# PolusAI/nyxus

Hardware: AMD Instinct MI355X
Metric: ROIs/sec (*ALL_GLCM*+*ALL_INTENSITY*, 1024^2 tiles) (higher is better)
Workload: dtype f64; 1 GPU; *ALL_GLCM*+*ALL_INTENSITY*, coarse_gray_depth=8, 4 angles, d=1, 1000 synthetic 1024x1024 tiles/GPU x 196 ROIs/tile (disk r=30, 2821 px, bbox 61x61), intensities U[1,4095]; reduce stage on pre-assembled ROI clouds resident in HBM; n_columns=185

## Files before the change

### nyxus_amd/csrc/nyxhip_dispatch.hip

```cpp
#include "nyxhip_ctx.h"

using namespace nyxhip;

namespace {

uint32_t align16(uint32_t v) { return (v + 15u) & ~15u; }

void gabor_filter(double* Gex, double f0, double sig2lam, double gamma, double theta, double fi, int n)
{
    const double lambda = 2 * M_PI / f0, cos_theta = cos(theta), sin_theta = sin(theta), sig = sig2lam * lambda;
    std::vector<double> tx(n + 1), ty(n + 1);
    tx[0] = (n % 2 > 0) ? -((n - 1) / 2) : -(n / 2);
    for (int x = 1; x < n; x++) tx[x] = tx[x - 1] + 1;
    ty[0] = tx[0];
    for (int y = 1; y < n; y++) ty[y] = ty[y - 1] + 1;
    double sum = 0;
    for (int y = 0; y < n; y++)
        for (int x = 0; x < n; x++) {
            double xte = tx[x] * cos_theta + ty[y] * sin_theta;
            double yte = ty[y] * cos_theta - tx[x] * sin_theta;
            double rte = xte * xte + gamma * gamma * yte * yte;
            double ge = exp(-1 * rte / (2 * sig * sig));
            double argm = xte * f0 + fi;
            int idx = y * n * 2 + x * 2;
// ... 1069 lines not shown
        const bool after_all = (mask & kBehindIntensity) && (mask & NYXHIP_FAM_GLCM);
        if (after_all) lane_join.join();
        if (int mrc = launch_contour_families(ctx, b, mask, s, d_out, ld, max_px, max_area, max_side, !after_all))
            return mrc;
    }
    return NYXHIP_OK;
}

}

namespace nyxhip {

int use_lane(nyxhip_ctx* ctx, int lane, hipStream_t* st)
{
    if (!ctx->lane_stream[lane]) {
        static const bool no_prio = [] { const char* e = getenv("NYXHIP_NO_LANE_PRIORITY"); return e && *e && *e != '0'; }();
        int lo = 0, hi = 0;
        if (no_prio || hipDeviceGetStreamPriorityRange(&lo, &hi) != hipSuccess) lo = hi = 0;
        HIP_TRY(ctx, hipStreamCreateWithPriority(&ctx->lane_stream[lane], hipStreamNonBlocking, hi));
        HIP_TRY(ctx, hipEventCreateWithFlags(&ctx->lane_done[lane], hipEventDisableTiming));
    }
    if (!ctx->lane_used[lane]) {
        HIP_TRY(ctx, hipStreamWaitEvent(ctx->lane_stream[lane], ctx->lane_fork, 0));
        ctx->lane_used[lane] = true;
    }
    *st = ctx->lane_stream[lane];
    return NYXHIP_OK;
}

size_t large_budget(size_t dflt)
{
    const char* const be = getenv("NYXHIP_LARGE_BUDGET_MB");
    return be && atoll(be) > 0 ? (size_t)atoll(be) << 20 : dflt;
}

uint32_t pow2ceil(uint32_t v)
{
    uint32_t p = 1;
    while (p < v) p <<= 1;
    return p;
}

int make_layout(uint32_t mask, const nyxhip_settings* s, int n_cols, uint32_t max_px, uint32_t max_area,
                uint32_t max_range, LdsLayout& L, std::string& why, size_t cap, uint32_t vmax, bool wide_only)
{
    memset(&L, 0, sizeof(L));
    const bool do_int = mask & NYXHIP_FAM_INTENSITY, do_glcm = mask & NYXHIP_FAM_GLCM;
    const bool spill = cap != 0;
    if (!spill) cap = roi_features_max_lds();
    uint32_t off = 0;
    L.out = off;
    L.red = off; off = align16(off + 8u * kWaves * 8);
    L.stat = off; off = align16(off + 8u * 16);
    L.lb100 = off; off = align16(off + 4u * 104);
    uint32_t n_hist = (uint32_t)abs(s->grey_depth);
    L.lbc = off; off = align16(off + 4u * (do_int ? n_hist + 8 : 8));
    const uint32_t fixed = off;
    const uint32_t kCountCapMax = spill ? (1u << 22) : 16384u, kCountCapMixed = 4096;
    const bool radix = do_int && wide_only && !spill;
    if (radix) {
        L.count_cap = 0;
        L.sort_cap = max_px ? max_px : 1;
    } else if (do_int) {
        if ((uint64_t)max_range + 1 <= kCountCapMax) {
            L.count_cap = (max_range + 1 + 63u) & ~63u;
            L.sort_cap = max_px ? max_px : 1;
        } else {
            L.count_cap = kCountCapMixed;
            L.sort_cap = pow2ceil(max_px ? max_px : 1);
        }
    }
    L.dense_cap = do_glcm ? max_area : 0;
    L.dense = off;
    {
        const int gi = s->ibsi ? 0 : s->grey_depth;
        const bool c16_pred = do_int && max_px < 65536u && (uint64_t)max_range + 1 <= kCountCapMax && max_range < 65536u;
        const bool split_pred = do_glcm && !spill && gi > 0 && gi <= 16 && s->glcm_n_angles > 0;
        L.dense8 = ((c16_pred || !do_int) && split_pred) ? 1u : 0u;
    }
    {
        const int gi = s->ibsi ? 0 : s->grey_depth;
        const bool c16_pred = (!do_int || (uint64_t)max_range + 1 <= kCountCapMax) && max_range < 65536u;
        L.g16 = (do_glcm && !spill && gi > 16 && gi <= 64 && max_px < 32768u && c16_pred && s->glcm_n_angles > 0) ? 1u : 0u;
        if (L.g16) L.dense8 = 1;
    }
    if ((L.dense8 ? 1ull : 2ull) * L.dense_cap > cap) { why = "ROI bounding box of " + std::to_string(max_area) + " px exceeds the LDS-resident plane"; return NYXHIP_ERR_ROI_TOO_LARGE; }
    uint32_t plane_bytes = L.dense8 ? 1u * L.dense_cap + 64 + 8 : 2u * L.dense_cap + 8;
    const uint32_t g16_scratch = L.g16 ? 8u * ((uint32_t)s->grey_depth + kMaxAngles * 128u) : 0u;
    if (plane_bytes < g16_scratch) plane_bytes = g16_scratch;
    off = align16(off + plane_bytes);
    if (do_glcm) {
        const int greyInfo = s->ibsi ? 0 : s->grey_depth;
        L.lvl_cap = greyInfo < 0 ? (uint32_t)(-greyInfo) : 0;
        L.lvlmap = off; off = align16(off + 2u * (L.lvl_cap + 8));
    }
    const uint32_t shared0 = off;
    L.val = off;
    L.cnt16 = (do_int && max_px < 65536u && (uint64_t)max_range + 1 <= kCountCapMax && max_range < 65536u) ? 1u : 0u;
    L.radix_k16 = (radix && max_range < 65536u) ? 1u : 0u;
    if ((L.cnt16 ? 2ull : 4ull) * L.sort_cap > cap) { why = "ROI pixel count " + std::to_string(max_px) + " exceeds the LDS-resident value buffer"; return NYXHIP_ERR_ROI_TOO_LARGE; }
    if (L.radix_k16) off = align16(off + 2u * 2u * ((L.sort_cap + 7u) & ~7u) + 16);
    else off = align16(off + (L.cnt16 ? 2u : 4u) * L.sort_cap + 16);
    L.cnt = off; off = align16(off + (L.cnt16 ? 2u : 4u) * L.count_cap + 16);
    if (radix) {
        if (8ull * L.sort_cap > cap) { why = "ROI pixel count " + std::to_string(max_px) + " exceeds the LDS-resident sort buffers"; return NYXHIP_ERR_ROI_TOO_LARGE; }
        L.radix = off; off = align16(off + (L.radix_k16 ? 0u : 4u * L.sort_cap) + 4u * (kWaves * 256 + kWaves) + 16);
    }
    if (do_glcm && L.g16) {
        const uint32_t ng = (uint32_t)s->grey_depth, cellsw = ((ng + 1) * ((ng + 3) & ~1u)) / 2;
        L.ng_cap = ng; L.app = 4;
        uint32_t goff = shared0;
        L.P = goff; goff = align16(goff + 4u * 4u * cellsw);
        L.gscr = L.dense;
        if (goff > off) off = goff;
    } else if (do_glcm) {
        const int greyInfo = s->ibsi ? 0 : s->grey_depth;
        auto glcm_bytes = [&](uint32_t ng, uint32_t app) -> size_t {
            return (size_t)align16(4u * app * ng * ng) + 8ull * (25ull * ng + 128);
        };
        uint32_t ng;
        if (greyInfo != 0) {
            ng = (uint32_t)abs(greyInfo);
            if (fixed + 2ull * (L.lvl_cap + 8) + glcm_bytes(ng, 1) > cap) {
                why = "GLCM grey depth " + std::to_string(ng) + " too large for the LDS-resident co-occurrence matrix";
                return NYXHIP_ERR_UNSUPPORTED;
            }
        } else {
            if (vmax != 0) {
                ng = vmax < 8 ? 8 : vmax;
                if (shared0 + glcm_bytes(ng, 1) > cap) {
                    why = "IBSI GLCM matrix order " + std::to_string(ng) + " too large for the LDS-resident co-occurrence matrix";
                    return NYXHIP_ERR_UNSUPPORTED;
                }
            } else {
                ng = 128;
                while (ng > 8 && shared0 + glcm_bytes(ng, 1) > cap) ng >>= 1;
            }
        }
        uint32_t app = 4;
        while (app > 1 && ((!spill && 4ull * app * ng * ng > 64 * 1024) || shared0 + glcm_bytes(ng, app) > cap)) app >>= 1;
        L.ng_cap = ng;
        L.app = app;
        uint32_t goff = shared0;
        L.P = goff; goff = align16(goff + 4u * app * (ng <= 16 ? (ng + 1) * (ng + 1) : ng * ng));
        L.gscr = goff; goff = align16(goff + 8u * (25u * ng + 128));
        if (goff > off) off = goff;
    }
    if (L.dense8) {
        const uint32_t dsz = align16(plane_bytes);
        L.out += dsz; L.red += dsz; L.stat += dsz; L.lb100 += dsz; L.lbc += dsz;
        L.dense = 0;
        if (L.g16) L.gscr = 0;
    }
    if (spill) {
        const uint32_t esz = L.cnt16 ? 2u : 4u;
        const uint64_t sz_val = align16(esz * L.sort_cap + 16), sz_cnt = do_int ? (uint64_t)esz * L.count_cap + 32 : 0;
        const uint64_t sz_dense = 2ull * L.dense_cap + 24, sz_lvl = do_glcm ? 2ull * (L.lvl_cap + 8) + 16 : 0;
        const uint64_t ngc = L.ng_cap, sz_P = do_glcm ? 4ull * L.app * (ngc <= 16 ? (ngc + 1) * (ngc + 1) : ngc * ngc) + 16 : 0;
        const uint64_t sz_g = do_glcm ? 8ull * (25ull * ngc + 128) + 16 : 0;
        const uint64_t kLdsMax = 60 * 1024;
        uint64_t o = fixed;
        const bool p_lds = do_glcm && o + sz_P + sz_g <= kLdsMax;
        if (p_lds) { L.P = (uint32_t)o; o = (o + sz_P + 15) & ~15ull; L.gscr = (uint32_t)o; o = (o + sz_g + 15) & ~15ull; }
        const bool c_lds = do_int && o + sz_cnt <= kLdsMax;
        if (c_lds) { L.cnt = (uint32_t)o; o = (o + sz_cnt + 15) & ~15ull; }
        const bool l_lds = do_glcm && o + sz_lvl <= kLdsMax;
        if (l_lds) { L.lvlmap = (uint32_t)o; o = (o + sz_lvl + 15) & ~15ull; }
        L.gs_lds_bytes = (uint32_t)o;
        if (do_glcm && !l_lds) { L.lvlmap = (uint32_t)o; o = (o + sz_lvl + 15) & ~15ull; }
        L.dense = (uint32_t)o; o = (o + sz_dense + 15) & ~15ull;
        L.val = (uint32_t)o; o = (o + sz_val + 15) & ~15ull;
        if (do_int && !c_lds) { L.cnt = (uint32_t)o; o = (o + sz_cnt + 15) & ~15ull; }
        if (do_glcm && !p_lds) { L.P = (uint32_t)o; o = (o + sz_P + 15) & ~15ull; L.gscr = (uint32_t)o; o = (o + sz_g + 15) & ~15ull; }
        if (o > cap) { why = "ROI too large for the global workspace (2 GiB of offsets per workgroup)"; return NYXHIP_ERR_ROI_TOO_LARGE; }
        off = (uint32_t)o;
    }
    L.total = off;
    if (L.total > cap) {
        why = "ROI too large for the LDS-resident path (" + std::to_string(L.total) + " B of LDS needed; max_px=" +
              std::to_string(max_px) + ", max_bbox_area=" + std::to_string(max_area) + ")";
        return NYXHIP_ERR_ROI_TOO_LARGE;
    }
    return NYXHIP_OK;
}

int ensure_stage(nyxhip_ctx* ctx, size_t bytes)
{
    HIP_TRY(ctx, ctx->d_stage.reserve(bytes, nullptr, bytes + bytes / 4 + (1 << 20)));
    return NYXHIP_OK;
}

int check_status(nyxhip_ctx* ctx)
{
    int two[2] = {0, 0};
    HIP_TRY(ctx, hipMemcpy(two, ctx->d_status.p, 2 * sizeof(int), hipMemcpyDeviceToHost));
    const int st = two[0];
    if (ctx->census_pending) {
        ctx->census_small = (uint32_t)two[1]; ctx->census_total = ctx->census_pending; ctx->census_pending = 0;
    }
    if (two[1]) HIP_TRY(ctx, hipMemsetAsync(ctx->d_status.as<int>() + 1, 0, sizeof(int), ctx->stream()));
    if (st != 0) {
        int zero = 0;
        HIP_TRY(ctx, hipMemcpy(ctx->d_status.p, &zero, sizeof(int), hipMemcpyHostToDevice));
// ... 88 lines not shown
```

### nyxus_amd/csrc/roi_features.hip

```cpp
#include <hip/hip_runtime.h>
#include <type_traits>
#include <algorithm>
#include <cstdlib>
#include <cstdio>
#include "device_math.h"
#include "roi_kernel.h"
#include "launch_util.h"
#include "glcm_rows.h"
#include "glcm_w64.h"
#include "intensity_close.h"
#include "sort_lds.h"
#include "../../include/nyxhip.h"

namespace nyxhip {


enum { S_MEAN = 0, S_P10, S_P90, S_MEDIAN, S_MODE, S_NG };


template <int NW> __device__ __forceinline__ double xw_chain(const double* s_red, int k)
{
    return NW == 1 ? s_red[k] : ((s_red[k] + s_red[8 + k]) + s_red[16 + k]) + s_red[24 + k];
}
template <int NW> __device__ __forceinline__ double xw_pairs(const double* s_red, int k)
// ... 642 lines not shown
    glcm_w64_tail<NG>(Ng, lane, rc, cc, dc, pxpy_c, csum, sum_p, inv_sum_p, pcol, prow, pxmy, pxpy, ent, hxy1c, hxy2, asm_i, cmax, f);
}

#ifdef NYX_STAMP
#define STAMP(i)                                                                          \
    do {                                                                                  \
        unsigned long long t__ = __builtin_readcyclecounter();                            \
        if (tid == 0 && A.stamps) atomicAdd(&A.stamps[i], t__ - t_prev__);                \
        t_prev__ = __builtin_readcyclecounter();                                          \
    } while (0)
#elif defined(NYX_EXIT_AT)
#define STAMP(i) do { if ((i) == NYX_EXIT_AT) return; } while (0)
#else
#define STAMP(i) do { } while (0)
#endif

__constant__ const double kPctFrac[8] = {0.01, 0.1, 0.25, 0.75, 0.9, 0.99, 0.5, 0.5};

typedef __attribute__((address_space(3))) uint8_t lds_u8_t;

typedef const __attribute__((address_space(4))) RoiArgs KArgs;
__device__ __forceinline__ KArgs* late_kernarg()
{
    KArgs* p = (KArgs*)__builtin_amdgcn_kernarg_segment_ptr();
    asm volatile("" : "+s"(p));
    return p;
}
template <bool LATE>
struct KView {
    const RoiArgs& a;
    KArgs* p;
    __device__ __forceinline__ explicit KView(const RoiArgs& a_) : a(a_), p(LATE ? late_kernarg() : nullptr) {}
    __device__ __forceinline__ auto operator->() const
    {
        if constexpr (LATE) return p;
        else return &a;
    }
};
template <bool GS, bool C16, bool SPLIT, bool D8, int FAM = 0, int TIER = 4, bool G16 = false, int WIN = 2, int NW = 4, bool DEFER_P = false>
__device__ __forceinline__ void roi_features_body(const RoiArgs& A, const uint64_t slot)
{
    static_assert((NW == 4 && NW == kMaxAngles) || (NW == 8 && G16 && FAM == 4), "one workgroup of four waves per ROI (and a wave per GLCM angle)");
    constexpr int BS = NW * 64;
    extern __shared__ __attribute__((aligned(16))) unsigned char lds_raw[];
    unsigned char* const lds = GS ? A.sp.scratch + (size_t)blockIdx.x * A.sp.stride : lds_raw;
    const int tid = (int)threadIdx.x, lane = tid & 63, wave = __builtin_amdgcn_readfirstlane(tid >> 6);
    uint64_t roi;
    if (!roi_of_slot(A.sp, slot, A.n_roi, roi))
        return;

    auto reg = [&](uint32_t o) -> unsigned char* { return (GS && o < A.L.gs_lds_bytes) ? lds_raw + o : lds + o; };
    double* s_red = (double*)reg(A.L.red);
    double* s_stat = (double*)reg(A.L.stat);
    uint32_t* s_lb100 = (uint32_t*)reg(A.L.lb100);
    uint32_t* s_lbc = (uint32_t*)reg(A.L.lbc);
    uint32_t* s_val = (uint32_t*)(lds + A.L.val);
    using dense_t = typename std::conditional<D8, uint8_t, uint16_t>::type;
    dense_t* s_dense = (dense_t*)(lds + (D8 ? 0u : A.L.dense));
    uint16_t* s_lvlmap = (uint16_t*)reg(A.L.lvlmap);
    uint32_t* s_P = (uint32_t*)reg(A.L.P);
    double* s_g = (double*)reg(A.L.gscr);

    const uint64_t off = A.px_offset[roi];
    const uint32_t n = (uint32_t)(A.px_offset[roi + 1] - off);
    const uint32_t w = A.bbox_w[roi], h = A.bbox_h[roi];
    const uint32_t area = w * h;
    const uint32_t vmin = A.min_inten[roi], vmax = A.max_inten[roi];
    if (!roi_in_launch(A.sp, n, w, h, vmax - vmin))
        return;
    if (vmax - vmin < A.sp.min_range || (A.sp.max_range != 0u && vmax - vmin > A.sp.max_range))
        return;
    constexpr bool FAST = FAM == 1 || FAM == 3;
    constexpr int kRowsTag = 16 + TIER * 4 + (C16 ? 2 : 0) + (D8 ? 1 : 0);
    const bool do_int = FAM == 1 || FAM == 2 || (FAM == 0 && (A.mask & NYXHIP_FAM_INTENSITY) != 0);
    const bool do_glcm = FAM == 1 || FAM == 3 || FAM == 4 || (FAM == 0 && (A.mask & NYXHIP_FAM_GLCM) != 0);
    double* const out_row = A.out + roi * A.ld;
#ifdef NYX_STAMP
    unsigned long long t_prev__ = __builtin_readcyclecounter();
#endif

    const uint32_t range = vmax - vmin;
    const bool use_count = C16 ? do_int : (do_int && A.L.count_cap != 0 && range < A.L.count_cap);
    if (C16 && do_int && range >= A.L.count_cap) {
        if (tid == 0) atomicCAS(A.status, 0, NYXHIP_ERR_ROI_TOO_LARGE);
        return;
    }
    uint32_t* s_cnt = (uint32_t*)reg(A.L.cnt);
    uint32_t P2 = 1;
    while (P2 < n)
        P2 <<= 1;
    const bool radix = !C16 && A.L.radix != 0;
    const bool k16 = radix && A.L.radix_k16 != 0;
    if (n == 0 || (do_int && ((use_count || radix) ? n : P2) > A.L.sort_cap) || (do_glcm && area > A.L.dense_cap)) {
        if (SPLIT && A.glcm_ng && tid == 0)
            A.glcm_ng[roi] = 0;
        if (n != 0 && A.sp.defer_large)
            return;
        if (tid == 0 && n != 0)
            atomicCAS(A.status, 0, NYXHIP_ERR_ROI_TOO_LARGE);
        for (int c = tid; c < A.n_cols; c += BS)
            out_row[c] = __longlong_as_double(0x7ff8000000000000LL);
        return;
    }

    const int greyInfo = A.ibsi ? 0 : A.grey_depth;
    if (FAST) __builtin_assume(greyInfo > 0 && greyInfo <= 16);
    if (G16) __builtin_assume(greyInfo > 16 && greyInfo <= 64);
// ... 277 lines not shown
        if ((unsigned long long)n * vmax < (1ull << 32))
            sum = wave_sum_t<uint32_t>((uint32_t)sum);
        else
            sum = wave_sum_u64(sum);
        if (C16) {
            const uint32_t lo24 = wave_sum_t<uint32_t>((uint32_t)sumsq & 0xFFFFFFu), hi = wave_sum_t<uint32_t>((uint32_t)(sumsq >> 24));
            sumsq = ((unsigned long long)hi << 24) + lo24;
        } else
            sumsq = wave_sum_u64(sumsq);
        if (lane == 0) {
            s_red[wave * 8 + 0] = (double)sum;
            s_red[wave * 8 + 1] = (double)sumsq;
        }
        grp_sync<GS, NW>();
        const bool blank = (vmin == 0 && vmax == 0);
#if defined(NYX_NO_FUSED) || defined(NYX_NO_DEFER)
        constexpr bool DEFER = false;
#else
        constexpr bool DEFER = DEFER_P && C16 && !GS;
#endif
        const bool defer = DEFER && !blank;
        double* const rec = DEFER ? B->close_rec + roi * kCloseRec : nullptr;
        if (tid == 0) {
            double tot = 0, totsq = 0;
            for (int wv = 0; wv < NW; wv++) {
                tot += s_red[wv * 8 + 0];
                totsq += s_red[wv * 8 + 1];
            }
            const double mean = tot / dn;
            s_stat[S_MEAN] = mean;
            if (FAST)
                s_stat[S_NG] = bin_pixel(vmin, vmin, vmax, B->glcm_grey_depth) == bin_pixel(vmax, vmin, vmax, B->glcm_grey_depth) ? 1.0 : 0.0;
            if (defer) {
                rec[CR_TOT] = tot;
                rec[CR_TOTSQ] = totsq;
            } else {
                close_sums(RowColumns{o}, dn, vmin, vmax, tot, totsq, mean, B->slide_min && B->slide_max,
                           [&] { return B->slide_max[roi] - B->slide_min[roi]; }, blank);
            }
        }
        grp_sync<GS, NW>();
        const double mean = s_stat[S_MEAN];
        STAMP(2);

        const double binW100 = (double)range / 100.;
        const uint32_t nb = (uint32_t)B->n_hist;
        auto idx100 = [=](uint32_t v) -> int {
            double realIdx = (double)(v - vmin) / binW100;
            return (realIdx != realIdx) ? 0 : (int)realIdx;
        };

        const uint32_t Q = ((range + 1 + NW * 512 - 1) / (NW * 512)) * 512;
        uint32_t* const s_woff = (uint32_t*)(s_stat + 8);
        if (use_count) {
            uint32_t carry = 0, best_c = 0, best_i = 0;
            const uint32_t base = wave * Q;
            if (C16) {
                uint32_t kk[8] = {0, 0, 0, 0, 0, 0, 0, 0};
                uint32_t inv = 0xFFFFu - (base + 8u * (uint32_t)lane);
                uint4* src = (uint4*)((uint16_t*)s_cnt + base + 8u * (uint32_t)lane);
                uint32_t i = base + 8u * (uint32_t)lane;
                for (uint32_t t = 0; t < Q; t += 512, i += 512, inv -= 512, src += 64) {
                    uint4 pk = make_uint4(0, 0, 0, 0);
                    const bool live = i <= range;
                    if (live) pk = *src;
                    kk[0] = max(kk[0], (pk.x << 16) | inv); kk[1] = max(kk[1], (pk.x & 0xFFFF0000u) | inv);
                    kk[2] = max(kk[2], (pk.y << 16) | inv); kk[3] = max(kk[3], (pk.y & 0xFFFF0000u) | inv);
                    kk[4] = max(kk[4], (pk.z << 16) | inv); kk[5] = max(kk[5], (pk.z & 0xFFFF0000u) | inv);
                    kk[6] = max(kk[6], (pk.w << 16) | inv); kk[7] = max(kk[7], (pk.w & 0xFFFF0000u) | inv);
                    const uint32_t A0 = pk.x + (pk.x << 16), A1 = pk.y + (pk.y << 16), A2 = pk.z + (pk.z << 16), A3 = pk.w + (pk.w << 16);
                    const uint32_t T = ((A0 + A1) + (A2 + A3)) >> 16;
                    const uint32_t sc = wave_scan_u32(T);
                    const uint32_t excl = carry + sc - T;
                    const uint32_t o0 = A0 + (excl | (excl << 16));
                    const uint32_t o1 = A1 + __builtin_amdgcn_perm(o0, o0, 0x03020302u);
                    const uint32_t o2 = A2 + __builtin_amdgcn_perm(o1, o1, 0x03020302u);
                    const uint32_t o3 = A3 + __builtin_amdgcn_perm(o2, o2, 0x03020302u);
                    if (live)
                        *src = make_uint4(o0, o1, o2, o3);
                    carry += readlane63(sc);
                }
#pragma unroll
                for (int q = 1; q < 8; q++) kk[q] -= (uint32_t)q;
                const uint32_t key = wave_max_u32(max(max(max(kk[0], kk[1]), max(kk[2], kk[3])), max(max(kk[4], kk[5]), max(kk[6], kk[7]))));
                best_c = key >> 16;
                best_i = 0xFFFFu - (key & 0xFFFFu);
            } else
            for (uint32_t t = 0; t < Q; t += 256) {
                uint32_t i = base + t + 4 * lane;
                uint4 c4 = make_uint4(0, 0, 0, 0);
                if (C16) {
                    if (i <= range) {
                        const uint2 pk = *(const uint2*)((const uint16_t*)s_cnt + i);
                        c4 = make_uint4(pk.x & 0xFFFFu, pk.x >> 16, pk.y & 0xFFFFu, pk.y >> 16);
                    }
                } else if (i + 3 <= range)
                    c4 = *(const uint4*)&s_cnt[i];
                else {
                    if (i <= range) c4.x = s_cnt[i];
                    if (i + 1 <= range) c4.y = s_cnt[i + 1];
                    if (i + 2 <= range) c4.z = s_cnt[i + 2];
                }
                if (c4.x > best_c) { best_c = c4.x; best_i = i; }
                if (c4.y > best_c) { best_c = c4.y; best_i = i + 1; }
                if (c4.z > best_c) { best_c = c4.z; best_i = i + 2; }
                if (c4.w > best_c) { best_c = c4.w; best_i = i + 3; }
                c4.y += c4.x; c4.z += c4.y; c4.w += c4.z;
                const uint32_t sc = wave_scan_u32(c4.w);
                uint32_t excl = carry + sc - c4.w;
                c4.x += excl; c4.y += excl; c4.z += excl; c4.w += excl;
                if (C16) {
                    if (i <= range)
                        *(uint2*)((uint16_t*)s_cnt + i) = make_uint2(c4.x | (c4.y << 16), c4.z | (c4.w << 16));
                } else if (i + 3 <= range)
                    *(uint4*)&s_cnt[i] = c4;
                else {
                    if (i <= range) s_cnt[i] = c4.x;
                    if (i + 1 <= range) s_cnt[i + 1] = c4.y;
                    if (i + 2 <= range) s_cnt[i + 2] = c4.z;
                }
                carry += readlane63(sc);
            }
            if (!C16) {
                const uint32_t mc_w = wave_max_u32(best_c);
                const uint32_t cand = best_c == mc_w ? best_i : 0xFFFFFFFFu;
                best_i = ~wave_max_u32(~cand);
                best_c = mc_w;
            }
            if (lane == 0) {
                s_red[wave * 8 + 0] = (double)carry;
                s_red[wave * 8 + 1] = (double)best_c;
                s_red[wave * 8 + 2] = (double)best_i;
            }
            grp_sync<GS, NW>();
            if (tid == 0) {
                uint32_t mc = 0, mi = 0;
                for (int wv = 0; wv < NW; wv++) {
                    uint32_t c = (uint32_t)s_red[wv * 8 + 1], i = (uint32_t)s_red[wv * 8 + 2];
                    if (c > mc) { mc = c; mi = i; }
                }
                const uint32_t woff1 = (uint32_t)s_red[0], woff2 = woff1 + (NW > 1 ? (uint32_t)s_red[8] : 0u), woff3 = woff2 + (NW > 1 ? (uint32_t)s_red[16] : 0u);
                s_woff[0] = 0; s_woff[1] = woff1; s_woff[2] = woff2; s_woff[3] = woff3;
                s_stat[S_MODE] = (double)(vmin + mi);
            }
            grp_sync<GS, NW>();
        } else if (radix) {
            if (k16) {
                uint16_t* const kb = (uint16_t*)s_val + ((B->L.sort_cap + 7u) & ~7u);
                s_val = (uint32_t*)radix_sort<GS, NW, uint16_t>((uint16_t*)s_val, kb, (uint32_t*)reg(B->L.radix), n, 0u, range, tid);
            } else {
                uint32_t* const s_rdx = (uint32_t*)reg(B->L.radix);
                s_val = radix_sort<GS, NW, uint32_t>(s_val, s_rdx, s_rdx + B->L.sort_cap, n, vmin, range, tid);
            }
        } else {
            bitonic_sort<GS, NW>(s_val, P2, tid);
        }
        STAMP(3);
        auto SV = [=](uint32_t i) -> uint32_t { return k16 ? vmin + (uint32_t)((const uint16_t*)s_val)[i] : s_val[i]; };
        auto cum = [=](uint32_t i) -> uint32_t {
            const uint32_t wq = (uint32_t)(i >= Q) + (uint32_t)(i >= 2 * Q) + (uint32_t)(i >= 3 * Q);
            return (C16 ? (uint32_t)((const uint16_t*)s_cnt)[i] : s_cnt[i]) + s_woff[wq];
        };

#ifdef NYX_NO_FUSED
        constexpr bool FUSED = false;
#else
        constexpr bool FUSED = C16 && !GS;
#endif
        double acc[6] = {0, 0, 0, 0, 0, 0};
        if (!FUSED || blank) {
            if (!blank) {
                for (uint32_t i = tid; i < n; i += BS) {
                    double d = (double)(C16 ? vmin + ((const uint16_t*)s_val)[i] : SV(i)) - mean;
                    double d2 = d * d;
                    acc[0] += fabs(d);
                    acc[1] += d2;
                    acc[2] += d2 * d;
                    acc[3] += d2 * d2;
                    acc[4] += d2 * d2 * d;
                    acc[5] += d2 * d2 * d2;
                }
                block_sum<6, GS, NW>(acc, s_red, tid);
            }
            if (tid == 0)
                close_central<CovDiv::ieee>(RowColumns{o}, acc, n, dn, mean, blank);
        }
        STAMP(4);

        if (!blank) {
            auto bin_bound = [&](auto is100_t, const uint32_t b) -> uint32_t {
                constexpr bool is100 = decltype(is100_t)::value;
                uint32_t lo;
                if (use_count) {
                    auto bin_of = [=](uint32_t dd) -> uint32_t {
                        return is100 ? (uint32_t)idx100(vmin + dd) : to_grayscale(vmin + dd, vmin, range, nb);
                    };
                    uint32_t d;
                    if (range < 65536u) {
                        const double Wl = is100 ? binW100 : (double)range / (double)nb;
                        const double P = (double)b * Wl;
                        const uint32_t m = (uint32_t)(P + 0.5);
                        d = (uint32_t)P + 1;
                        if (b == 0)
                            d = 0;
                        else if (fabs(P - (double)m) < 1e-6)
                            d = bin_of(m) >= b ? m : m + 1;
                    } else {
                        double edge = is100 ? (double)b * binW100 : (double)b * (double)range / (double)nb;
                        d = edge >= (double)range + 1.0 ? range + 1 : (uint32_t)edge;
                        while (d > 0 && bin_of(d - 1) >= b) d--;
                        while (d <= range && bin_of(d) < b) d++;
                    }
                    lo = d > 0 ? cum(d - 1) : 0u;
                } else {
                    uint32_t hi = n;
                    lo = 0;
                    while (lo < hi) {
                        uint32_t mid = (lo + hi) >> 1;
                        uint32_t v = SV(mid);
                        uint32_t idx = is100 ? (uint32_t)idx100(v) : to_grayscale(v, vmin, range, nb);
                        if (idx < b) lo = mid + 1; else hi = mid;
// ... 23 lines not shown
                for (int d = 32; d > 0; d >>= 1) {
                    uint32_t oc = __shfl_down(best_c, d, 64), ov = __shfl_down(best_v, d, 64);
                    if (oc > best_c || (oc == best_c && ov < best_v)) { best_c = oc; best_v = ov; }
                }
                if (lane == 0) {
                    s_red[wave * 8 + 0] = (double)best_c;
                    s_red[wave * 8 + 1] = (double)best_v;
                }
                grp_sync<GS, NW>();
                if (tid == 0) {
                    uint32_t mc = 0, mv = 0;
                    for (int wv = 0; wv < NW; wv++) {
                        uint32_t c = (uint32_t)s_red[wv * 8 + 0], v = (uint32_t)s_red[wv * 8 + 1];
                        if (c > mc || (c == mc && v < mv)) { mc = c; mv = v; }
                    }
                    s_stat[S_MODE] = (double)mv;
                }
            }
            STAMP(6);

            if (NW == 1 || wave == 0) {
                const int g = lane >> 3, sub = lane & 7;
                const double mycnt = dn * kPctFrac[g];
                const uint32_t k = g < 6 ? (uint32_t)mycnt : (g == 6 || n / 2 == 0) ? n / 2 : n / 2 - 1;
                uint32_t xv;
                if (use_count) {
                    uint32_t lom1 = 0xFFFFFFFFu, span = range + 1;
                    while (span > 1) {
                        const uint32_t B = (span + 7) >> 3;
                        uint32_t i = mad_u24_su((uint32_t)sub + 1, B, lom1);
                        if (i > range) i = range;
                        const unsigned long long hit = __ballot(cum(i) > k);
                        const uint32_t half = lane < 32 ? (uint32_t)hit : (uint32_t)(hit >> 32);
                        const uint32_t first = (uint32_t)__builtin_ctz(((half >> (lane & 24)) & 0xFFu) | 0x80u);
                        lom1 = mad_u24_su(first, B, lom1);
                        span = B;
                    }
                    xv = vmin + lom1 + 1;
                } else
                    xv = SV(k);
                const uint32_t win = min((uint32_t)idx100(xv), 99u);
                const uint32_t bb = win + (uint32_t)sub;
                uint32_t bnd = 0;
                if (g < 6 && sub < 2)
                    bnd = bb < 100u ? bin_bound(std::true_type{}, bb) : n;
                const uint32_t rs = bnd, bi = wave_rol1(bnd) - rs;
                const double pv = (mycnt - (double)rs) * binW100 / (double)bi + (double)vmin + binW100 * (double)win;
                static_assert(I_P10 == I_P01 + 1 && I_P25 == I_P01 + 2 && I_P75 == I_P01 + 3 && I_P90 == I_P01 + 4 && I_P99 == I_P01 + 5, "P01 .. P99 are adjacent columns");
                if (g < 6 && sub == 0)
                    o[I_P01 + g] = pv;
                const double p10 = readlane_f64(pv, 8), p90 = readlane_f64(pv, 32);
                const double p25 = DEFER ? 0.0 : readlane_f64(pv, 16), p75 = DEFER ? 0.0 : readlane_f64(pv, 24);
                const uint32_t hi_v = (uint32_t)__builtin_amdgcn_readlane((int)xv, 48), lo_v = (uint32_t)__builtin_amdgcn_readlane((int)xv, 56);
                if (lane == 0) {
                    if (!DEFER)
                        close_quartiles(RowColumns{o}, p25, p75);
                    s_stat[S_P10] = p10;
                    s_stat[S_P90] = p90;
                    if (FUSED) {
                        uint32_t lox = 0x80000000u, span = 0;
                        if (p10 <= p90 && p90 >= (double)vmin && p10 <= (double)vmax) {
                            const double cl = ceil(p10), fl = floor(p90);
                            const uint32_t lo_b = cl <= (double)vmin ? vmin : (uint32_t)cl, hi_b = fl >= (double)vmax ? vmax : (uint32_t)fl;
                            if (lo_b <= hi_b) { lox = lo_b - vmin; span = hi_b - lo_b; }
                        }
                        const bool empty = span == 0 && lox == 0x80000000u;
                        uint32_t* const s_rob = (uint32_t*)(s_stat + 6);
                        s_rob[0] = lox;
                        s_rob[1] = span;
                        s_rob[2] = (empty || lox == 0) ? 0u : cum(lox - 1);
                        s_rob[3] = empty ? 0u : cum(lox + span);
                    }
                    double median = (n & 1) ? (double)hi_v : (double)(uint32_t)(hi_v + lo_v) / 2.0;
                    o[I_MEDIAN] = median;
                    o[I_MODE] = s_stat[S_MODE];
                    s_stat[S_MEDIAN] = median;
                    if (FUSED) {
                        const uint32_t m2x = (uint32_t)((median - (double)vmin) * 2.0);
                        uint32_t* const s_med = (uint32_t*)(s_stat + 10);
                        s_med[0] = m2x;
                        s_med[1] = (m2x & 1u) ? cum(m2x >> 1) : 0u;
                    }
                }
            }
            if (NW == 1 || wave == 1) {
                for (uint32_t b = lane; b < nb; b += 64)
                    s_lbc[b] = bin_bound(std::false_type{}, b);
                wav_sync<GS>();
                double e = 0, u = 0;
                for (uint32_t k = lane; k < nb; k += 64) {
                    uint32_t ck = (k < nb - 1 ? s_lbc[k + 1] : n) - s_lbc[k];
                    double p = fdiv((double)ck, dn);
                    e += p * log2(p + 2.2e-16);
                    u += p * p;
                }
                e = wave_sum(e);
                u = wave_sum(u);
                if (lane == 0) {
                    o[I_ENTROPY] = -e;
                    o[I_UNIFORMITY] = u;
                }
            }
            grp_sync<GS, NW>();
            STAMP(7);

            const double p10 = s_stat[S_P10], p90 = s_stat[S_P90], median = s_stat[S_MEDIAN];
            if (FUSED) {
                const uint32_t* const s_rob = (const uint32_t*)(s_stat + 6);
                const uint32_t lox = (uint32_t)__builtin_amdgcn_readfirstlane((int)s_rob[0]), span = (uint32_t)__builtin_amdgcn_readfirstlane((int)s_rob[1]);
                const uint32_t hix = lox + span;
                const uint32_t m2x = (uint32_t)__builtin_amdgcn_readfirstlane((int)((const uint32_t*)(s_stat + 10))[0]);
                const uint32_t kmed = m2x >> 1;
                uint32_t sx = 0, sad = 0;
                const double meanx = mean - (double)vmin;
                auto px1 = [&](uint32_t x) {
                    const double d = (double)x - meanx;
                    const double d2 = d * d;
                    acc[0] += fabs(d);
                    acc[1] = __builtin_fma(d, d, acc[1]);
                    acc[2] = __builtin_fma(d2, d, acc[2]);
                    acc[3] = __builtin_fma(d2, d2, acc[3]);
                    const double d4 = d2 * d2;
                    acc[4] = __builtin_fma(d4, d, acc[4]);
                    acc[5] = __builtin_fma(d4, d2, acc[5]);
                    sx += med3_u32_ss(x, lox, hix);
                    asm("v_sad_u32 %0, %1, %2, %0" : "+v"(sad) : "v"(x), "s"(kmed));
                };
                const uint16_t* const pv = (const uint16_t*)s_val + tid;
                const uint32_t n_full = (uint32_t)__builtin_amdgcn_readfirstlane((int)(n / BS)), n_rem = n - n_full * BS;
                {
                    uint32_t k = 0;
                    for (; k + 1 < n_full; k += 2) { px1(pv[k * BS]); px1(pv[(k + 1) * BS]); }
                    if (k < n_full) px1(pv[k * BS]);
                }
                if ((uint32_t)tid < n_rem)
                    px1(pv[n_full * BS]);
                {
                    const uint32_t wsx = wave_sum_t<uint32_t>(sx), wsad = wave_sum_t<uint32_t>(sad);
                    if (lane == 0) {
                        s_red[wave * 8 + 6] = (double)wsx;
                        s_red[wave * 8 + 7] = (double)wsad;
                    }
                }
                {
                    double t[8];
#pragma unroll
                    for (int k = 0; k < 8; k++) t[k] = k < 6 ? acc[k] : 0.0;
                    const double tot = wave_transpose_sum8(t, lane);
                    if ((lane & 7) == 0 && (lane >> 3) < 6)
                        s_red[wave * 8 + (lane >> 3)] = tot;
                }
                grp_sync<GS, NW>();
                const uint32_t n_below = (uint32_t)__builtin_amdgcn_readfirstlane((int)s_rob[2]);
                const uint32_t n_upto = (uint32_t)__builtin_amdgcn_readfirstlane((int)s_rob[3]);
                const uint32_t K = n_upto - n_below, n_above = n - n_upto;
                const uint32_t Sx_all = (uint32_t)xw_pairs<NW>(s_red, 6);
                const uint32_t Sxu = (uint32_t)__builtin_amdgcn_readfirstlane((int)(Sx_all - n_below * lox - n_above * hix));
                const double Sx = (double)Sxu;
                if (DEFER) {
                    if (tid < 8)
                        rec[CR_ACC + tid] = xw_chain<NW>(s_red, tid);
                    if (tid == 0) {
                        uint32_t* const rw = (uint32_t*)rec;
                        *(uint4*)(rw + CR_W_NBELOW) = make_uint4(n_below, n_above, K, Sxu);
                        *(uint4*)(rw + CR_W_LOX) = make_uint4(lox, hix, m2x, ((const uint32_t*)(s_stat + 10))[1]);
                    }
                } else
                if (tid == 0) {
                    double a6[6];
#pragma unroll
                    for (int k = 0; k < 6; k++) {
                        a6[k] = xw_chain<NW>(s_red, k);
                        asm volatile("" : "+v"(a6[k]) :: "memory");
                    }
                    const double sadk = xw_pairs<NW>(s_red, 7);
                    const uint32_t cle = ((const uint32_t*)(s_stat + 10))[1];
                    close_central<CovDiv::ieee>(RowColumns{o}, a6, n, dn, mean, blank);
                    close_robust_mad(RowColumns{o}, sadk, m2x, cle, K, Sx, vmin, dn);
                }
                const uint32_t Ku = K;
                const bool fast32 = (unsigned long long)(n_full + 1) * Ku * (span + 1ull) < (1ull << 32);
                double ad1[1];
                if (fast32) {
                    uint32_t ad = 0;
                    auto px2 = [&](uint32_t x) {
                        const uint32_t t = mul_u24_su(med3_u32_ss(x, lox, hix), Ku);
                        asm("v_sad_u32 %0, %1, %2, %0" : "+v"(ad) : "v"(t), "s"(Sxu));
                    };
                    {
                        uint32_t k = 0;
                        for (; k + 1 < n_full; k += 2) { px2(pv[k * BS]); px2(pv[(k + 1) * BS]); }
                        if (k < n_full) px2(pv[k * BS]);
                    }
                    if ((uint32_t)tid < n_rem)
                        px2(pv[n_full * BS]);
                    ad1[0] = (double)ad;
                } else {
                    unsigned long long ad = 0;
                    auto px2 = [&](uint32_t x) {
                        const uint32_t t = (uint32_t)__umul24(Ku, x);
                        uint32_t dlt;
                        asm("v_sad_u32 %0, %1, %2, 0" : "=v"(dlt) : "v"(t), "s"(Sxu));
                        ad += (x - lox) <= span ? dlt : 0u;
                    };
                    for (uint32_t k = 0; k < n_full; k++)
                        px2(pv[k * BS]);
                    if ((uint32_t)tid < n_rem)
                        px2(pv[n_full * BS]);
                    ad1[0] = (double)ad;
                }
                block_sum<1, GS, NW>(ad1, (double*)s_lb100, tid);
                if (DEFER) {
                    if (tid == 0) {
                        rec[CR_ADIN] = ad1[0];
                        ((uint32_t*)rec)[CR_W_FAST32] = fast32 ? 1u : 0u;
                        B->close_flag[roi] = 1u;
                    }
                } else
                if (tid == 0)
                    close_robust_rmad(RowColumns{o}, ad1[0], fast32, K, Sx, lox, hix, n_below, n_above);
            } else {
            double rb[3] = {0, 0, 0};
            for (uint32_t i = tid; i < n; i += BS) {
                double a = (double)(C16 ? vmin + ((const uint16_t*)s_val)[i] : SV(i));
                if (a >= p10 && a <= p90) {
                    rb[0] += a;
                    rb[1] += 1.0;
                }
                rb[2] += fabs(a - median);
            }
            block_sum<3, GS, NW>(rb, s_red, tid);
            const double mean1090 = rb[1] > 0 ? rb[0] / rb[1] : 0.0;
            double ad[1] = {0};
            for (uint32_t i = tid; i < n; i += BS) {
                double a = (double)(C16 ? vmin + ((const uint16_t*)s_val)[i] : SV(i));
                if (a >= p10 && a <= p90)
                    ad[0] += fabs(a - mean1090);
            }
            block_sum<1, GS, NW>(ad, s_red, tid);
            if (tid == 0) {
                o[I_ROBUST_MEAN] = mean1090;
                o[I_ROBUST_MEAN_ABSOLUTE_DEVIATION] = rb[1] > 0 ? ad[0] / rb[1] : 0.0;
                o[I_MEDIAN_ABSOLUTE_DEVIATION] = fdiv(rb[2], dn);
            }
            }
        }

        STAMP(8);
    }

    STAMP(9);
    if (FAST) {
        double* o = out_row_l + B->col_glcm;
        const int na = B->glcm_na;
        const int Ng = greyInfo, NG1 = Ng + 1, NN = Ng * Ng, cells = NG1 * NG1;
        const bool degenerate = FAM == 3 ? bin_pixel(vmin, vmin, vmax, B->glcm_grey_depth) == bin_pixel(vmax, vmin, vmax, B->glcm_grey_depth) : s_stat[S_NG] != 0.0;
        if (tid == 0)
            B->glcm_ng[roi] = degenerate ? 0u : (uint32_t)Ng;
        if (degenerate) {
            for (int c = tid; c < kGlcmAngled * na + kGlcmAve; c += BS)
                o[c] = 0.0;
            return;
        }
        const bool symmetric = B->glcm_symmetric != 0;
        int slot0 = -1, slot1 = -1, slot2 = -1, slot3 = -1;
#pragma unroll
        for (int q = 0; q < kMaxAngles; q++)
            if (q < na) {
                const int ang = B->glcm_angles[q];
                if (ang == 0) slot0 = q; else if (ang == 45) slot1 = q; else if (ang == 90) slot2 = q; else slot3 = q;
            }
        const bool usual = slot0 >= 0 && slot1 >= 0 && slot2 >= 0 && slot3 >= 0 && !symmetric;
        const bool dpp2 = B->glcm_offset == 1 && w > 64 && w <= 128 && usual;
        const bool dpp = (B->glcm_offset == 1 && w <= 64) || dpp2;
// ... 1096 lines not shown
```

### nyxus_amd/csrc/roi_kernel.h

```cpp
#pragma once
#include <stdint.h>
#include <stddef.h>
#include "../../include/nyxhip.h"

namespace nyxhip {

constexpr int kBlock = 256;
constexpr int kWaves = kBlock / 64;
constexpr int kIntensityCols = 36;
constexpr int kGlcmAngled = 30;
constexpr int kGlcmAve = 29;
constexpr int kMaxAngles = 4;

constexpr int kSizeClasses = 5, kClasses = 2 * kSizeClasses;
constexpr uint32_t kClassPx[kSizeClasses - 1] = {256, 4096, 16384, 32768};
constexpr uint32_t kClassSide[kSizeClasses - 1] = {32, 64, 128, 256};
constexpr uint32_t kLdsLevels = 128;
constexpr int kFirstLargeSizeClass = 3;
__host__ __device__ inline int roi_class(uint32_t n, uint32_t w, uint32_t h, uint32_t range, uint32_t lvl = 0)
{
    const uint32_t side = w > h ? w : h;
    int sc = (n <= 256u && side <= 32u) ? 0 : (n <= 4096u && side <= 64u) ? 1 : (n <= 16384u && side <= 128u) ? 2 : (n <= 32768u && side <= 256u) ? 3 : 4;
    if (sc == 2 && range >= 65536u) sc = 3;
    if (sc < 3 && lvl > kLdsLevels) sc = 3;
    const bool c16 = n < 65536u && range < 16384u;
    return 2 * sc + (c16 ? 0 : 1);
}
static_assert(kClassPx[0] == 256 && kClassPx[1] == 4096 && kClassPx[2] == 16384 && kClassPx[3] == 32768 && kClassSide[0] == 32 &&
              kClassSide[1] == 64 && kClassSide[2] == 128 && kClassSide[3] == 256, "roi_class spells the bounds out");

struct SpillArgs {
    const uint32_t* roi_index;
    unsigned char* scratch;
    uint64_t stride;
    int32_t defer_large;
    uint32_t n_slots;
    uint32_t class_mask;
    uint32_t min_range;
    uint32_t max_range;
    uint32_t skip_ltex;
};
__device__ __forceinline__ bool roi_in_launch(const SpillArgs& sp, uint32_t n, uint32_t w, uint32_t h, uint32_t range)
{
    return sp.class_mask == 0 || ((sp.class_mask >> roi_class(n, w, h, range)) & 1u) != 0;
}

__device__ __forceinline__ bool roi_of_slot(const SpillArgs& sp, uint64_t slot, uint64_t n_roi, uint64_t& roi)
{
    if (sp.roi_index) {
        if (slot >= sp.n_slots) return false;
        roi = sp.roi_index[slot];
    } else
        roi = slot;
    return roi < n_roi;
}

struct LdsLayout {
    uint32_t out;
    uint32_t red;
    uint32_t stat;
    uint32_t lb100;
    uint32_t lbc;
    uint32_t val;
    uint32_t cnt;
    uint32_t dense;
    uint32_t lvlmap;
    uint32_t P;
    uint32_t gscr;
    uint32_t total;
    uint32_t sort_cap;
    uint32_t count_cap;
    uint32_t cnt16;
    uint32_t dense8;
    uint32_t dense_cap;
    uint32_t ng_cap;
    uint32_t lvl_cap;
    uint32_t app;
    uint32_t g16;
    uint32_t gs_lds_bytes;
    uint32_t radix;
    uint32_t radix_k16;
};

struct WindowSrc {
    const void* inten;
    const void* lab;
    int32_t dt_inten, dt_label;
    uint32_t W, H;
    const uint32_t* tile;
    const uint32_t* label;
    const uint32_t* x0;
    const uint32_t* y0;
    uint32_t xcd_swz;
};
__host__ __device__ inline uint64_t xcd_slot(uint32_t b, uint32_t grid) { const uint32_t per = (grid + 7u) >> 3; return (uint64_t)(b & 7u) * per + (b >> 3); }

constexpr int kCloseRec = 16;
enum {
    CR_TOT = 0, CR_TOTSQ,
    CR_ACC,
    CR_SADK = 9,
    CR_ADIN,
    CR_W_FAST32 = 22,
    CR_W_NBELOW = 24, CR_W_NABOVE, CR_W_K, CR_W_SXU,
    CR_W_LOX, CR_W_HIX, CR_W_M2X, CR_W_CLE
};

struct RoiArgs {
    uint64_t n_roi;
    const uint64_t* px_offset;
    const uint16_t* x;
    const uint16_t* y;
    const uint32_t* inten;
    const uint32_t* bbox_w;
    const uint32_t* bbox_h;
    const uint32_t* min_inten;
    const uint32_t* max_inten;
    const double* slide_min;
    const double* slide_max;
    double* out;
    uint64_t ld;
    int* status;
    unsigned long long* stamps;
    uint32_t mask;
    int32_t n_cols;
// ... 450 lines not shown
```

Baseline: 102.2 million ROIs/s.

## Compute robust MAD stats from sparse first-moment prefix sums during count scan

While scanning the 16-bit intensity count histogram, the kernel now also builds a strided prefix sum of value-weighted counts (first moment) in LDS, with the stride chosen so LDS occupancy is not reduced. Trimmed-range sums, median absolute deviation and the inner robust MAD are then taken from a few prefix lookups instead of extra per-pixel passes and block reductions, including the second pixel pass and its block_sum. This adds udot2 work and a wave scan to the histogram loop, plus a new LDS region replacing the lb100 scratch buffer.

```diff
diff --git a/nyxus_amd/csrc/nyxhip_dispatch.hip b/nyxus_amd/csrc/nyxhip_dispatch.hip
--- a/nyxus_amd/csrc/nyxhip_dispatch.hip
+++ b/nyxus_amd/csrc/nyxhip_dispatch.hip
@@ -1145,7 +1145,6 @@
     L.out = off;
     L.red = off; off = align16(off + 8u * kWaves * 8);
     L.stat = off; off = align16(off + 8u * 16);
-    L.lb100 = off; off = align16(off + 4u * 104);
     uint32_t n_hist = (uint32_t)abs(s->grey_depth);
     L.lbc = off; off = align16(off + 4u * (do_int ? n_hist + 8 : 8));
     const uint32_t fixed = off;
@@ -1199,6 +1198,7 @@
         if (8ull * L.sort_cap > cap) { why = "ROI pixel count " + std::to_string(max_px) + " exceeds the LDS-resident sort buffers"; return NYXHIP_ERR_ROI_TOO_LARGE; }
         L.radix = off; off = align16(off + (L.radix_k16 ? 0u : 4u * L.sort_cap) + 4u * (kWaves * 256 + kWaves) + 16);
     }
+    const uint32_t cnt_end = off;
     if (do_glcm && L.g16) {
         const uint32_t ng = (uint32_t)s->grey_depth, cellsw = ((ng + 1) * ((ng + 3) & ~1u)) / 2;
         L.ng_cap = ng; L.app = 4;
@@ -1239,9 +1239,20 @@
         L.gscr = goff; goff = align16(goff + 8u * (25u * ng + 128));
         if (goff > off) off = goff;
     }
+    if (L.cnt16 && !spill) {
+        const uint32_t lds_cu = (uint32_t)roi_features_max_lds();
+        auto wgs = [&](uint32_t total) -> uint32_t { return std::min<uint32_t>(8u, lds_cu / (total ? total : 1u)); };
+        uint32_t sh = 3, with = off;
+        for (;; sh++) {
+            with = std::max(off, align16(cnt_end + 4u * ((L.count_cap + (1u << sh) - 1u) >> sh)));
+            if (sh == 9 || wgs(with) >= wgs(off)) break;
+        }
+        L.fm = cnt_end; L.fm_shift = sh;
+        off = with;
+    }
     if (L.dense8) {
         const uint32_t dsz = align16(plane_bytes);
-        L.out += dsz; L.red += dsz; L.stat += dsz; L.lb100 += dsz; L.lbc += dsz;
+        L.out += dsz; L.red += dsz; L.stat += dsz; L.lbc += dsz;
         L.dense = 0;
         if (L.g16) L.gscr = 0;
     }
diff --git a/nyxus_amd/csrc/roi_features.hip b/nyxus_amd/csrc/roi_features.hip
--- a/nyxus_amd/csrc/roi_features.hip
+++ b/nyxus_amd/csrc/roi_features.hip
@@ -718,7 +718,6 @@
     auto reg = [&](uint32_t o) -> unsigned char* { return (GS && o < A.L.gs_lds_bytes) ? lds_raw + o : lds + o; };
     double* s_red = (double*)reg(A.L.red);
     double* s_stat = (double*)reg(A.L.stat);
-    uint32_t* s_lb100 = (uint32_t*)reg(A.L.lb100);
     uint32_t* s_lbc = (uint32_t*)reg(A.L.lbc);
     uint32_t* s_val = (uint32_t*)(lds + A.L.val);
     using dense_t = typename std::conditional<D8, uint8_t, uint16_t>::type;
@@ -1102,6 +1101,13 @@
 
         const uint32_t Q = ((range + 1 + NW * 512 - 1) / (NW * 512)) * 512;
         uint32_t* const s_woff = (uint32_t*)(s_stat + 8);
+#ifdef NYX_NO_FUSED
+        constexpr bool FUSED = false;
+#else
+        constexpr bool FUSED = C16 && !GS;
+#endif
+        uint32_t* const s_fm = (uint32_t*)(lds + B->L.fm);
+        uint32_t* const s_foff = (uint32_t*)(s_stat + 12);
         if (use_count) {
             uint32_t carry = 0, best_c = 0, best_i = 0;
             const uint32_t base = wave * Q;
@@ -1110,6 +1116,9 @@
                 uint32_t inv = 0xFFFFu - (base + 8u * (uint32_t)lane);
                 uint4* src = (uint4*)((uint16_t*)s_cnt + base + 8u * (uint32_t)lane);
                 uint32_t i = base + 8u * (uint32_t)lane;
+                typedef unsigned short u16x2 __attribute__((ext_vector_type(2)));
+                uint32_t fcarry = 0;
+                const uint32_t fm_sh = FUSED ? B->L.fm_shift : 0u, fm_mask = (1u << fm_sh) - 1u;
                 for (uint32_t t = 0; t < Q; t += 512, i += 512, inv -= 512, src += 64) {
                     uint4 pk = make_uint4(0, 0, 0, 0);
                     const bool live = i <= range;
@@ -1129,7 +1138,20 @@
                     if (live)
                         *src = make_uint4(o0, o1, o2, o3);
                     carry += readlane63(sc);
-                }
+                    if (FUSED) {
+                        uint32_t qc = __builtin_amdgcn_udot2(__builtin_bit_cast(u16x2, pk.x), __builtin_bit_cast(u16x2, 0x00010000u), 0u, false);
+                        qc = __builtin_amdgcn_udot2(__builtin_bit_cast(u16x2, pk.y), __builtin_bit_cast(u16x2, 0x00030002u), qc, false);
+                        qc = __builtin_amdgcn_udot2(__builtin_bit_cast(u16x2, pk.z), __builtin_bit_cast(u16x2, 0x00050004u), qc, false);
+                        qc = __builtin_amdgcn_udot2(__builtin_bit_cast(u16x2, pk.w), __builtin_bit_cast(u16x2, 0x00070006u), qc, false);
+                        const uint32_t m = mad24(i, T, qc);
+                        const uint32_t fs = wave_scan_u32(m);
+                        if (live && (i & fm_mask) == 0)
+                            s_fm[i >> fm_sh] = fcarry + fs - m;
+                        fcarry += readlane63(fs);
+                    }
+                }
+                if (FUSED && lane == 0)
+                    s_red[wave * 8 + 3] = (double)fcarry;
 #pragma unroll
                 for (int q = 1; q < 8; q++) kk[q] -= (uint32_t)q;
                 const uint32_t key = wave_max_u32(max(max(max(kk[0], kk[1]), max(kk[2], kk[3])), max(max(kk[4], kk[5]), max(kk[6], kk[7]))));
@@ -1191,6 +1213,11 @@
                 }
                 const uint32_t woff1 = (uint32_t)s_red[0], woff2 = woff1 + (NW > 1 ? (uint32_t)s_red[8] : 0u), woff3 = woff2 + (NW > 1 ? (uint32_t)s_red[16] : 0u);
                 s_woff[0] = 0; s_woff[1] = woff1; s_woff[2] = woff2; s_woff[3] = woff3;
+                if (FUSED) {
+                    const uint32_t f1 = (uint32_t)s_red[3], f2 = f1 + (NW > 1 ? (uint32_t)s_red[8 + 3] : 0u), f3 = f2 + (NW > 1 ? (uint32_t)s_red[16 + 3] : 0u);
+                    s_foff[0] = 0; s_foff[1] = f1; s_foff[2] = f2; s_foff[3] = f3;
+                    s_foff[4] = f3 + (NW > 1 ? (uint32_t)s_red[24 + 3] : 0u);
+                }
                 s_stat[S_MODE] = (double)(vmin + mi);
             }
             grp_sync<GS, NW>();
@@ -1211,12 +1238,19 @@
             const uint32_t wq = (uint32_t)(i >= Q) + (uint32_t)(i >= 2 * Q) + (uint32_t)(i >= 3 * Q);
             return (C16 ? (uint32_t)((const uint16_t*)s_cnt)[i] : s_cnt[i]) + s_woff[wq];
         };
-
-#ifdef NYX_NO_FUSED
-        constexpr bool FUSED = false;
-#else
-        constexpr bool FUSED = C16 && !GS;
-#endif
+        auto fm_at = [=](uint32_t p, uint32_t sub) -> uint32_t {
+            const uint32_t fm_sh = B->L.fm_shift;
+            const uint32_t wq = (uint32_t)(p >= Q) + (uint32_t)(p >= 2 * Q) + (uint32_t)(p >= 3 * Q);
+            const uint32_t q0 = mul24(wq, Q);
+            const uint16_t* const c16 = (const uint16_t*)s_cnt;
+            uint32_t part = 0;
+            for (uint32_t j = ((p >> fm_sh) << fm_sh) + sub; j <= p; j += 8) {
+                const uint32_t cj = c16[j], pj = j == q0 ? 0u : (uint32_t)c16[j == 0 ? 0 : j - 1];
+                part = mad24(j, cj - pj, part);
+            }
+            return grp8_sum(part) + s_fm[p >> fm_sh] + s_foff[wq];
+        };
+
         double acc[6] = {0, 0, 0, 0, 0, 0};
         if (!FUSED || blank) {
             if (!blank) {
@@ -1346,34 +1380,58 @@
                 const double p10 = readlane_f64(pv, 8), p90 = readlane_f64(pv, 32);
                 const double p25 = DEFER ? 0.0 : readlane_f64(pv, 16), p75 = DEFER ? 0.0 : readlane_f64(pv, 24);
                 const uint32_t hi_v = (uint32_t)__builtin_amdgcn_readlane((int)xv, 48), lo_v = (uint32_t)__builtin_amdgcn_readlane((int)xv, 56);
+                const double median = (n & 1) ? (double)hi_v : (double)(uint32_t)(hi_v + lo_v) / 2.0;
                 if (lane == 0) {
                     if (!DEFER)
                         close_quartiles(RowColumns{o}, p25, p75);
-                    s_stat[S_P10] = p10;
-                    s_stat[S_P90] = p90;
-                    if (FUSED) {
-                        uint32_t lox = 0x80000000u, span = 0;
-                        if (p10 <= p90 && p90 >= (double)vmin && p10 <= (double)vmax) {
-                            const double cl = ceil(p10), fl = floor(p90);
-                            const uint32_t lo_b = cl <= (double)vmin ? vmin : (uint32_t)cl, hi_b = fl >= (double)vmax ? vmax : (uint32_t)fl;
-                            if (lo_b <= hi_b) { lox = lo_b - vmin; span = hi_b - lo_b; }
-                        }
-                        const bool empty = span == 0 && lox == 0x80000000u;
-                        uint32_t* const s_rob = (uint32_t*)(s_stat + 6);
-                        s_rob[0] = lox;
-                        s_rob[1] = span;
-                        s_rob[2] = (empty || lox == 0) ? 0u : cum(lox - 1);
-                        s_rob[3] = empty ? 0u : cum(lox + span);
-                    }
-                    double median = (n & 1) ? (double)hi_v : (double)(uint32_t)(hi_v + lo_v) / 2.0;
                     o[I_MEDIAN] = median;
                     o[I_MODE] = s_stat[S_MODE];
-                    s_stat[S_MEDIAN] = median;
-                    if (FUSED) {
-                        const uint32_t m2x = (uint32_t)((median - (double)vmin) * 2.0);
-                        uint32_t* const s_med = (uint32_t*)(s_stat + 10);
-                        s_med[0] = m2x;
-                        s_med[1] = (m2x & 1u) ? cum(m2x >> 1) : 0u;
+                    if (!FUSED) {
+                        s_stat[S_P10] = p10;
+                        s_stat[S_P90] = p90;
+                        s_stat[S_MEDIAN] = median;
+                    }
+                }
+                if (FUSED) {
+                    uint32_t lox = 0x80000000u, span = 0;
+                    if (p10 <= p90 && p90 >= (double)vmin && p10 <= (double)vmax) {
+                        const double cl = ceil(p10), fl = floor(p90);
+                        const uint32_t lo_b = cl <= (double)vmin ? vmin : (uint32_t)cl, hi_b = fl >= (double)vmax ? vmax : (uint32_t)fl;
+                        if (lo_b <= hi_b) { lox = lo_b - vmin; span = hi_b - lo_b; }
+                    }
+                    const bool empty = span == 0 && lox == 0x80000000u, has_lo = !empty && lox != 0;
+                    const uint32_t hix = lox + span;
+                    const uint32_t m2x = (uint32_t)((median - (double)vmin) * 2.0), kmed = m2x >> 1;
+                    const uint32_t pt = g == 0 ? (has_lo ? lox - 1 : 0u) : g == 1 ? (empty ? 0u : hix) : kmed;
+                    const uint32_t fv = fm_at(pt, (uint32_t)sub), cv = cum(pt);
+                    const uint32_t n_below = has_lo ? (uint32_t)__builtin_amdgcn_readlane((int)cv, 0) : 0u;
+                    const uint32_t F_lo = has_lo ? (uint32_t)__builtin_amdgcn_readlane((int)fv, 0) : 0u;
+                    const uint32_t n_upto = empty ? 0u : (uint32_t)__builtin_amdgcn_readlane((int)cv, 8);
+                    const uint32_t F_hi = empty ? 0u : (uint32_t)__builtin_amdgcn_readlane((int)fv, 8);
+                    const uint32_t Ck = (uint32_t)__builtin_amdgcn_readlane((int)cv, 16), Fk = (uint32_t)__builtin_amdgcn_readlane((int)fv, 16);
+                    const uint32_t K = n_upto - n_below, n_above = n - n_upto, Sxu = F_hi - F_lo;
+                    const uint32_t sadk_u = (kmed * Ck - Fk) + ((s_foff[4] - Fk) - kmed * (n - Ck));
+                    unsigned long long adin_u = 0;
+                    if (K != 0) {
+                        const uint32_t t = min((uint32_t)((double)Sxu / (double)K), range);
+                        const uint32_t ft = (uint32_t)__builtin_amdgcn_readfirstlane((int)fm_at(t, (uint32_t)sub));
+                        const uint32_t n1 = (uint32_t)__builtin_amdgcn_readfirstlane((int)cum(t)) - n_below, S1 = ft - F_lo;
+                        adin_u = 2ull * ((unsigned long long)Sxu * n1 - (unsigned long long)K * S1);
+                    }
+                    if (lane == 0) {
+                        const uint32_t cle = (m2x & 1u) ? Ck : 0u;
+                        const double sadk = (double)sadk_u, adin = (double)adin_u, Sx = (double)Sxu;
+                        if (DEFER) {
+                            uint32_t* const rw = (uint32_t*)rec;
+                            rec[CR_SADK] = sadk;
+                            rec[CR_ADIN] = adin;
+                            rw[CR_W_FAST32] = 0u;
+                            *(uint4*)(rw + CR_W_NBELOW) = make_uint4(n_below, n_above, K, Sxu);
+                            *(uint4*)(rw + CR_W_LOX) = make_uint4(lox, hix, m2x, cle);
+                        } else {
+                            close_robust_mad(RowColumns{o}, sadk, m2x, cle, K, Sx, vmin, dn);
+                            close_robust_rmad(RowColumns{o}, adin, false, K, Sx, lox, hix, n_below, n_above);
+                        }
                     }
                 }
             }
@@ -1398,14 +1456,7 @@
             grp_sync<GS, NW>();
             STAMP(7);
 
-            const double p10 = s_stat[S_P10], p90 = s_stat[S_P90], median = s_stat[S_MEDIAN];
             if (FUSED) {
-                const uint32_t* const s_rob = (const uint32_t*)(s_stat + 6);
-                const uint32_t lox = (uint32_t)__builtin_amdgcn_readfirstlane((int)s_rob[0]), span = (uint32_t)__builtin_amdgcn_readfirstlane((int)s_rob[1]);
-                const uint32_t hix = lox + span;
-                const uint32_t m2x = (uint32_t)__builtin_amdgcn_readfirstlane((int)((const uint32_t*)(s_stat + 10))[0]);
-                const uint32_t kmed = m2x >> 1;
-                uint32_t sx = 0, sad = 0;
                 const double meanx = mean - (double)vmin;
                 auto px1 = [&](uint32_t x) {
                     const double d = (double)x - meanx;
@@ -1417,8 +1468,6 @@
                     const double d4 = d2 * d2;
                     acc[4] = __builtin_fma(d4, d, acc[4]);
                     acc[5] = __builtin_fma(d4, d2, acc[5]);
-                    sx += med3_u32_ss(x, lox, hix);
-                    asm("v_sad_u32 %0, %1, %2, %0" : "+v"(sad) : "v"(x), "s"(kmed));
                 };
                 const uint16_t* const pv = (const uint16_t*)s_val + tid;
                 const uint32_t n_full = (uint32_t)__builtin_amdgcn_readfirstlane((int)(n / BS)), n_rem = n - n_full * BS;
@@ -1430,13 +1479,6 @@
                 if ((uint32_t)tid < n_rem)
                     px1(pv[n_full * BS]);
                 {
-                    const uint32_t wsx = wave_sum_t<uint32_t>(sx), wsad = wave_sum_t<uint32_t>(sad);
-                    if (lane == 0) {
-                        s_red[wave * 8 + 6] = (double)wsx;
-                        s_red[wave * 8 + 7] = (double)wsad;
-                    }
-                }
-                {
                     double t[8];
 #pragma unroll
                     for (int k = 0; k < 8; k++) t[k] = k < 6 ? acc[k] : 0.0;
@@ -1445,75 +1487,25 @@
                         s_red[wave * 8 + (lane >> 3)] = tot;
                 }
                 grp_sync<GS, NW>();
-                const uint32_t n_below = (uint32_t)__builtin_amdgcn_readfirstlane((int)s_rob[2]);
-                const uint32_t n_upto = (uint32_t)__builtin_amdgcn_readfirstlane((int)s_rob[3]);
-                const uint32_t K = n_upto - n_below, n_above = n - n_upto;
-                const uint32_t Sx_all = (uint32_t)xw_pairs<NW>(s_red, 6);
-                const uint32_t Sxu = (uint32_t)__builtin_amdgcn_readfirstlane((int)(Sx_all - n_below * lox - n_above * hix));
-                const double Sx = (double)Sxu;
                 if (DEFER) {
-                    if (tid < 8)
+                    if (tid < 6)
                         rec[CR_ACC + tid] = xw_chain<NW>(s_red, tid);
+                    if (tid == 0)
+                        B->close_flag[roi] = 1u;
+                } else {
                     if (tid == 0) {
-                        uint32_t* const rw = (uint32_t*)rec;
-                        *(uint4*)(rw + CR_W_NBELOW) = make_uint4(n_below, n_above, K, Sxu);
-                        *(uint4*)(rw + CR_W_LOX) = make_uint4(lox, hix, m2x, ((const uint32_t*)(s_stat + 10))[1]);
-                    }
-                } else
-                if (tid == 0) {
-                    double a6[6];
-#pragma unroll
-                    for (int k = 0; k < 6; k++) {
-                        a6[k] = xw_chain<NW>(s_red, k);
-                        asm volatile("" : "+v"(a6[k]) :: "memory");
-                    }
-                    const double sadk = xw_pairs<NW>(s_red, 7);
-                    const uint32_t cle = ((const uint32_t*)(s_stat + 10))[1];
-                    close_central<CovDiv::ieee>(RowColumns{o}, a6, n, dn, mean, blank);
-                    close_robust_mad(RowColumns{o}, sadk, m2x, cle, K, Sx, vmin, dn);
-                }
-                const uint32_t Ku = K;
-                const bool fast32 = (unsigned long long)(n_full + 1) * Ku * (span + 1ull) < (1ull << 32);
-                double ad1[1];
-                if (fast32) {
-                    uint32_t ad = 0;
-                    auto px2 = [&](uint32_t x) {
-                        const uint32_t t = mul_u24_su(med3_u32_ss(x, lox, hix), Ku);
-                        asm("v_sad_u32 %0, %1, %2, %0" : "+v"(ad) : "v"(t), "s"(Sxu));
-                    };
-                    {
-                        uint32_t k = 0;
-                        for (; k + 1 < n_full; k += 2) { px2(pv[k * BS]); px2(pv[(k + 1) * BS]); }
-                        if (k < n_full) px2(pv[k * BS]);
-                    }
-                    if ((uint32_t)tid < n_rem)
-                        px2(pv[n_full * BS]);
-                    ad1[0] = (double)ad;
-                } else {
-                    unsigned long long ad = 0;
-                    auto px2 = [&](uint32_t x) {
-                        const uint32_t t = (uint32_t)__umul24(Ku, x);
-                        uint32_t dlt;
-                        asm("v_sad_u32 %0, %1, %2, 0" : "=v"(dlt) : "v"(t), "s"(Sxu));
-                        ad += (x - lox) <= span ? dlt : 0u;
-                    };
-                    for (uint32_t k = 0; k < n_full; k++)
-                        px2(pv[k * BS]);
-                    if ((uint32_t)tid < n_rem)
-                        px2(pv[n_full * BS]);
-                    ad1[0] = (double)ad;
-                }
-                block_sum<1, GS, NW>(ad1, (double*)s_lb100, tid);
-                if (DEFER) {
-                    if (tid == 0) {
-                        rec[CR_ADIN] = ad1[0];
-                        ((uint32_t*)rec)[CR_W_FAST32] = fast32 ? 1u : 0u;
-                        B->close_flag[roi] = 1u;
-                    }
-                } else
-                if (tid == 0)
-                    close_robust_rmad(RowColumns{o}, ad1[0], fast32, K, Sx, lox, hix, n_below, n_above);
+                        double a6[6];
+#pragma unroll
+                        for (int k = 0; k < 6; k++) {
+                            a6[k] = xw_chain<NW>(s_red, k);
+                            asm volatile("" : "+v"(a6[k]) :: "memory");
+                        }
+                        close_central<CovDiv::ieee>(RowColumns{o}, a6, n, dn, mean, blank);
+                    }
+                    grp_sync<GS, NW>();
+                }
             } else {
+            const double p10 = s_stat[S_P10], p90 = s_stat[S_P90], median = s_stat[S_MEDIAN];
             double rb[3] = {0, 0, 0};
             for (uint32_t i = tid; i < n; i += BS) {
                 double a = (double)(C16 ? vmin + ((const uint16_t*)s_val)[i] : SV(i));
diff --git a/nyxus_amd/csrc/roi_kernel.h b/nyxus_amd/csrc/roi_kernel.h
--- a/nyxus_amd/csrc/roi_kernel.h
+++ b/nyxus_amd/csrc/roi_kernel.h
@@ -59,7 +59,7 @@
     uint32_t out;
     uint32_t red;
     uint32_t stat;
-    uint32_t lb100;
+    uint32_t fm;
     uint32_t lbc;
     uint32_t val;
     uint32_t cnt;
@@ -71,6 +71,7 @@
     uint32_t sort_cap;
     uint32_t count_cap;
     uint32_t cnt16;
+    uint32_t fm_shift;
     uint32_t dense8;
     uint32_t dense_cap;
     uint32_t ng_cap;
```

Result: faster. 104.1 million ROIs/s, median of 6 (+1.8%).
